# SudeepDasari/visual_foresight

Hardware: AMD Instinct MI355X
Metric: predicted frames/sec (whole node), 200-sample x 13-step x 64x64 CEM (higher is better)
Workload: dtype f32

## Files before the change

visual_foresight_amd/csrc/vf_conv_mfma.h:

```cpp
#pragma once
#include <hip/hip_runtime.h>
#include <type_traits>

#ifdef VF_HOST_SELFTEST
#define VF_GLOBAL __device__
#define VF_LAUNCH_BOUNDS(...)
#else
#define VF_GLOBAL __global__
#define VF_LAUNCH_BOUNDS(...) __launch_bounds__(__VA_ARGS__)
#endif

namespace vf {

constexpr int kPollSleep = 16;

#ifdef VF_TILE_STATS
__device__ unsigned long long g_tile_clk[32][8];
#define VF_TS_NOW() (threadIdx.x == 0 ? wall_clock64() : 0ull)
#define VF_TS_ADD(KEY_, SLOT_, DT_) do { if (threadIdx.x == 0) atomicAdd(&g_tile_clk[KEY_][SLOT_], (unsigned long long)(DT_)); } while (0)
#else
#define VF_TS_NOW() 0ull
#define VF_TS_ADD(KEY_, SLOT_, DT_) do { } while (0)
#endif

// ... 822 lines not shown
}

template <class PT>
__device__ __forceinline__ void conv_pair_epilogue(const PT &p, f32x16 (&acc)[1][2], const int bx, float *smem) {
    typedef const __attribute__((address_space(4))) ConvParams QT;
    const unsigned long long qa = reinterpret_cast<unsigned long long>(p.fuse_next);
    const unsigned qlo = __builtin_amdgcn_readfirstlane((unsigned)qa);
    const unsigned qhi = __builtin_amdgcn_readfirstlane((unsigned)(qa >> 32));
    QT &q = *(QT *)(((unsigned long long)qhi << 32) | qlo);
    const int tid = threadIdx.x, lane = tid & 63, wave = tid >> 6;
    const int n = lane & 31, kh = lane >> 5;
    constexpr int KCP = 36;
    const int bimg0 = bx * p.NI;
    float *T = smem;

    const int Ntot = q.ncg * 32;
    const float *wl = q.Wp + ((long long)kh * Ntot + n) * 4;
    const long long wstep = (long long)2 * Ntot * 4;
    f32x4 wb[2][4][2];
#pragma unroll
    for (int c = 0; c < 2; ++c)
#pragma unroll
        for (int k8 = 0; k8 < 4; ++k8)
#pragma unroll
            for (int g = 0; g < 2; ++g)
                wb[c][k8][g] = *reinterpret_cast<const f32x4 *>(wl + (long long)(c * 4 + k8) * wstep + g * 128);

    __syncthreads();
#pragma unroll
    for (int g = 0; g < 2; ++g) {
        const float bias = p.bias[g * 32 + n];
#pragma unroll
        for (int r = 0; r < 16; ++r) {
            const int row = wave * 32 + (r & 3) + 8 * (r >> 2) + 4 * kh;
            T[(g * 128 + row) * KCP + n] = fmaxf(acc[0][g][r] + bias, 0.f);
        }
    }
    __syncthreads();

    f32x16 acc2[2];
#pragma unroll
    for (int g = 0; g < 2; ++g)
#pragma unroll
        for (int r = 0; r < 16; ++r) acc2[g][r] = 0.f;
    const f32x4 *T4 = reinterpret_cast<const f32x4 *>(T);
    const int arow = wave * 32 + n;
#pragma unroll
    for (int c = 0; c < 2; ++c)
#pragma unroll
        for (int k8 = 0; k8 < 4; ++k8) {
            const f32x4 a = T4[((c * 128 + arow) * KCP + k8 * 8 + kh * 4) >> 2];
#pragma unroll
            for (int j = 0; j < 4; ++j)
#pragma unroll
                for (int g = 0; g < 2; ++g)
                    acc2[g] = __builtin_amdgcn_mfma_f32_32x32x2f32(a[j], wb[c][k8][g][j], acc2[g], 0, 0, 0);
        }

    const int px_per_img = q.TH * q.TW;
    const long long out_elems = (long long)q.Hout * q.Wout * q.Cout;
    const TileDiv div_rpi(q.RPI), div_tw(q.TW);
#pragma unroll
    for (int g = 0; g < 2; ++g) {
        const int ch = g * 32 + n;
        const float bias = q.bias[g * 32 + n];
#pragma unroll
        for (int r = 0; r < 16; ++r) {
            const int row = wave * 32 + (r & 3) + 8 * (r >> 2) + 4 * kh;
            const int img = div_rpi.div(row), rem = row - img * q.RPI;
            const int y = div_tw.div(rem), x = rem - y * q.TW;
            const int b = bimg0 + img;
            if (!(img < q.NI && rem < px_per_img && b < q.B && y < q.Hout && x < q.Wout && ch < q.Cout)) continue;
            float v = acc2[g][r] + bias;
            if (q.sbias) v += q.sbias[(long long)b * q.sbias_ld + ch];
            v = fmaxf(v, 0.f);
            (q.out + (long long)b * out_elems)[(unsigned)((y * q.Wout + x) * q.Cout + ch)] = v;
        }
    }
}

template <int ND, bool FIRST, int K, class PT>
__device__ __forceinline__ void convt_fused_epilogue(const PT &p, f32x16 (&acc)[1][4], int bx, long long *red, float *smem);

template <int G, int EPI, int MREP, class PT, int RB = 4>
__device__ __forceinline__ void conv_tile(const PT &p, const int bx_, const int by_, const int bz_,
                                          float *smem) {
    const int bx = __builtin_amdgcn_readfirstlane(bx_), by = __builtin_amdgcn_readfirstlane(by_),
              bz = __builtin_amdgcn_readfirstlane(bz_);
    constexpr bool SPLIT = RB == 1 || RB == 2;
    [[maybe_unused]] constexpr bool kInLaunch = !std::is_same<PT, ConvParams>::value;
    constexpr bool GSPLIT = RB <= 0;
    static_assert(RB == 4 || (G == 4 && EPI == EPI_LSTM && ((SPLIT && MREP == 1) || RB == 0 || (RB == -2 && MREP == 1))),
                  "the row-split and gate-split tiles are conv-LSTM tiles");
    constexpr int MR = RB == 0 ? 4 * MREP : (RB < 0 ? -RB : MREP);
    constexpr int WROWS = MR * 32;
    constexpr int GA = GSPLIT ? 1 : (SPLIT ? RB : G);
    constexpr bool kBRing = SPLIT && RB == 1;
    constexpr bool kBLds = (EPI == EPI_LSTM) && MREP == 1 && !kBRing && !GSPLIT;
    const int tid = threadIdx.x, lane = tid & 63, wave = tid >> 6;
    const int n = lane & 31, kh = lane >> 5;
    const int wrow0 = GSPLIT ? 0 : (SPLIT ? (wave % RB) * 32 : wave * WROWS);
    const int gbase = GSPLIT ? wave : (SPLIT ? (wave / RB) * GA : 0);
    const int KC = p.KC, KCpad = KC + 4, K8 = KC >> 3;
    const int LH = (p.TH - 1) * p.stride + p.KH, LW = (p.TW - 1) * p.stride + p.KW;
    const int tile_px = LH * LW;
    const int tile_floats = p.NI * tile_px * KCpad;
    float *lnTab = smem + tile_floats;
    long long *red = reinterpret_cast<long long *>(lnTab + 4 * p.NI);
    const int cg = by;
    const int tiles_per_img = p.tilesY * p.tilesX;

    int bimg0, ty0, tx0, tile_id;
    if (p.NI == 1) {
        bimg0 = bx / tiles_per_img;
        tile_id = bx % tiles_per_img;
        ty0 = (tile_id / p.tilesX) * p.TH;
        tx0 = (tile_id % p.tilesX) * p.TW;
    } else {
        bimg0 = bx * p.NI;
        tile_id = 0; ty0 = 0; tx0 = 0;
    }

    [[maybe_unused]] const unsigned long long ts0 = VF_TS_NOW();
    [[maybe_unused]] unsigned long long ts1 = 0, ts_stage = 0;
    [[maybe_unused]] int ts_key = (((p.seg[0].C + (p.nseg > 1 ? p.seg[1].C : 0)) >> 5) & 7) + (p.Hout >= 32 ? 0 : 8);
    if constexpr (EPI == EPI_RAW_STATS) ts_key = 16;
    else if constexpr (EPI == EPI_BIAS_RELU) ts_key = p.KH == 1 ? 17 : (p.seg[0].C == 32 ? 18 : 19);
    else if constexpr (EPI == EPI_CONVT_RELU) ts_key = p.nseg == 1 ? 20 : 21;
    else if constexpr (EPI == EPI_PARTIAL) ts_key = 22;
    else if constexpr (is_top_fused(EPI)) ts_key = 23;
    else if constexpr (EPI == EPI_CONVT_RAW_STATS) ts_key = 24;
    const bool late = p.late_cnt != nullptr;
    ln_table(p, bimg0, lnTab, 0, late ? 1 : 2);
    [[maybe_unused]] const bool yielding = kInLaunch && EPI == EPI_LSTM && (GSPLIT || (SPLIT && RB == 1)) && late &&
                                           p.cu_state != nullptr && p.yield_budget > 0;
    [[maybe_unused]] int ybudget = p.yield_budget;
    [[maybe_unused]] const int *yword = yielding ? cu_partner_word(p) : nullptr;

    const int px_per_img = p.TH * p.TW;
    int abase[MR];
    {
        const TileDiv div_rpi(p.RPI), div_tw(p.TW);
#pragma unroll
        for (int m = 0; m < MR; ++m) {
            const int row = wrow0 + m * 32 + n;
            const int img = div_rpi.div(row), rem = row - img * p.RPI;
            const bool ok = img < p.NI && rem < px_per_img;
            const int y = div_tw.div(rem), x = rem - y * p.TW;
            abase[m] = (ok ? (img * tile_px + y * p.stride * LW + x * p.stride) * KCpad : 0) + kh * 4;
        }
    }

    f32x16 acc[MR][GA];
#pragma unroll
    for (int m = 0; m < MR; ++m)
#pragma unroll
        for (int g = 0; g < GA; ++g)
#pragma unroll
            for (int r = 0; r < 16; ++r) acc[m][g][r] = 0.f;

    const int ntaps = p.KH * p.KW;
    const int Ntot = p.ncg * G * 32;
    const int total_chunks = p.seg[0].nchunk + (p.nseg > 1 ? p.seg[1].nchunk : 0);
    const int ch_begin = bz * p.chunks_per_split;
    const int ch_end = min(ch_begin + p.chunks_per_split, total_chunks);
    const float *wlane = p.Wp + ((long long)kh * Ntot + (cg * G) * 32 + n) * 4;
    const long long wstep = (long long)2 * Ntot * 4;

    const int q4 = KC >> 2;
    const int q4_log2 = 31 - __builtin_clz((unsigned)q4);
    const unsigned magic_px = 0xFFFFFFFFu / (unsigned)tile_px + 1u, magic_lw = 0xFFFFFFFFu / (unsigned)LW + 1u;
    const int items = p.NI * tile_px * q4;

    constexpr bool kGbTab = EPI == EPI_LSTM;
    const int gbC = kGbTab ? ((p.seg[0].C + (p.nseg > 1 ? p.seg[1].C : 0) + 3) & ~3) : 0;
    float *gbTab = lnTab + 4 * p.NI + 16;
    if constexpr (kGbTab) {
        for (int i = tid; i < gbC; i += kConvThreads) {
            const int sgi = i < p.seg[0].C ? 0 : 1;
            const int cc = sgi ? i - p.seg[0].C : i;
            float g = 1.f, b = 0.f;
            if (sgi < p.nseg && cc < p.seg[sgi].C && p.seg[sgi].ln_part) {
                const int m = cc % p.seg[sgi].gamma_mod;
                g = p.seg[sgi].gamma[m]; b = p.seg[sgi].beta[m];
            }
            gbTab[i] = g; gbTab[gbC + i] = b;
        }
    }
    f32x4 *bsm = reinterpret_cast<f32x4 *>(gbTab + 2 * gbC);
    const float *wgate = p.Wp + ((long long)kh * Ntot + (cg * G + (wave & (G - 1))) * 32 + n) * 4;
    const int gt0 = ch_begin * ntaps, gtN = ch_end * ntaps;
    f32x4 breg[4];
#define VF_LOADB(GT_)                                                                           \
    _Pragma("unroll") for (int q = 0; q < 4; ++q)                                               \
        if (q < K8) breg[q] = *reinterpret_cast<const f32x4 *>(wgate + ((long long)(GT_) * K8 + q) * wstep);
#define VF_WRITEB(BUF_)                                                                         \
    _Pragma("unroll") for (int q = 0; q < 4; ++q)                                               \
        if (q < K8) bsm[(((BUF_) * K8 + q) * 4 + wave) * 64 + lane] = breg[q];
    if constexpr (kBLds) {
        if (gt0 < gtN) { VF_LOADB(gt0) }
    }
    [[maybe_unused]] f32x4 gsA[GSPLIT ? 4 : 1], gsB[GSPLIT ? 4 : 1];
    [[maybe_unused]] int gs_par = 0;
    [[maybe_unused]] const unsigned gs_loff = (unsigned)(((kh * Ntot + (cg * G + wave) * 32 + n) * 4) * 4);
    [[maybe_unused]] const unsigned gs_wstep_b = (unsigned)wstep * 4u;
    [[maybe_unused]] const __amdgpu_buffer_rsrc_t gs_rsrc =
        __builtin_amdgcn_make_buffer_rsrc(const_cast<float *>(p.Wp), 0, 0x7FFFFFFF, 0x00020000);
    if constexpr (GSPLIT) {
        if (gt0 < gtN) {
#pragma unroll
            for (int q = 0; q < 4; ++q)
                gsA[q] = __builtin_bit_cast(f32x4, __builtin_amdgcn_raw_buffer_load_b128(
                    gs_rsrc, gs_loff, (unsigned)(gt0 * 4 + q) * gs_wstep_b, 0));
        }
    }
    constexpr int kRing = 5;
    [[maybe_unused]] f32x4 bring[kBRing ? kRing : 1][kBRing ? 4 : 1][GA];
    [[maybe_unused]] const float *wring = p.Wp + ((long long)kh * Ntot + (cg * G + gbase) * 32 + n) * 4;
#define VF_LOADRING(SLOT_, GT_)                                                                 \
    _Pragma("unroll") for (int q_ = 0; q_ < 4; ++q_)                                            \
        _Pragma("unroll") for (int g_ = 0; g_ < GA; ++g_)                                       \
            bring[SLOT_][q_][g_] = *reinterpret_cast<const f32x4 *>(                            \
                wring + ((long long)(GT_) * 4 + q_) * wstep + g_ * 128);
    if constexpr (kBRing) {
#pragma unroll
        for (int d = 0; d < kRing; ++d)
            if (gt0 + d < gtN) { VF_LOADRING(d, gt0 + d) }
    }

    constexpr bool kGRing = EPI != EPI_LSTM;
    constexpr bool kConvT = (EPI == EPI_CONVT_RELU || EPI == EPI_CONVT_RAW_STATS || is_top_fused(EPI));
    [[maybe_unused]] f32x4 gring[kGRing ? (G == 1 ? 5 : 4) : 1][G];
    [[maybe_unused]] const int nit_g = ntaps * K8;
    [[maybe_unused]] const int ring_d = (nit_g & 3) == 0 ? 4 : ((G == 1 && nit_g % 5 == 0) ? 5 : 0);
#define VF_TAPLIVE(TAP_) (kConvT ? ((((TAP_) >= p.KW) ? 15 : 3) & ((((TAP_) % p.KW) != 0) ? 15 : 5)) : 15)
    [[maybe_unused]] const unsigned gr_loff = (unsigned)(((kh * Ntot + (cg * G) * 32 + n) * 4) * 4);
    [[maybe_unused]] const unsigned gr_wstep_b = (unsigned)wstep * 4u;
    [[maybe_unused]] const __amdgpu_buffer_rsrc_t gr_rsrc =
        __builtin_amdgcn_make_buffer_rsrc(const_cast<float *>(p.Wp), 0, 0x7FFFFFFF, 0x00020000);
#define VF_GLOAD(SLOT_, CI_, IT_)                                                               \
    {                                                                                           \
        const unsigned so_ = (unsigned)((CI_) * nit_g + (IT_)) * gr_wstep_b;                    \
        _Pragma("unroll") for (int g_ = 0; g_ < G; ++g_)                                        \
            gring[SLOT_][g_] = __builtin_bit_cast(f32x4, __builtin_amdgcn_raw_buffer_load_b128( \
                gr_rsrc, gr_loff, so_ + 512u * g_, 0));                                          \
    }
    if constexpr (kGRing) {
        if (ch_begin < ch_end) {
            if (ring_d == 4) {
#pragma unroll
                for (int d = 0; d < 4; ++d) VF_GLOAD(d, ch_begin, d)
            } else if (G == 1 && ring_d == 5) {
#pragma unroll
                for (int d = 0; d < 5; ++d) VF_GLOAD(d, ch_begin, d)
            } else if (G == 2) {
#pragma unroll
                for (int d = 0; d < 2; ++d) VF_GLOAD(d, ch_begin, d)
            }
        }
    }

    if constexpr (EPI == EPI_LSTM) __builtin_amdgcn_s_setprio(0);
    constexpr int kStageU = 4;
    for (int ci = ch_begin; ci < ch_end; ++ci) {
        const int s = (ci < p.seg[0].nchunk) ? 0 : 1;
        const auto &sg = p.seg[s];
        const int c0 = (s == 0 ? ci : ci - p.seg[0].nchunk) * KC;
        const bool vec_ok = (sg.C & 3) == 0;

        if (late && ci == p.seg[0].nchunk) {
            const int b1 = p.NI == 1 ? bimg0 + 1 : min(bimg0 + p.NI, p.B);
            if constexpr (kInLaunch) VF_TRACE_EVT(TR_LATE);
            if (!late_wait(p, bimg0, b1, reinterpret_cast<int *>(red))) return;
            if constexpr (kInLaunch) VF_TRACE_EVT(TR_LATE_END);
            ln_table(p, bimg0, lnTab, 1, 2);
        }
        __syncthreads();
        if constexpr (kInLaunch) VF_TRACE_EVT(TR_STAGE);
        [[maybe_unused]] const unsigned long long ts_s0 = VF_TS_NOW();
        constexpr bool kHoistLn = EPI != EPI_LSTM || MREP > 1;
        const int q = tid & (q4 - 1);
        const int c = c0 + 4 * q;
        const int nvalid = min(4, sg.C - c);
        const bool lean = vec_ok && sg.C % KC == 0;
        [[maybe_unused]] float gam[4] = {1.f, 1.f, 1.f, 1.f}, bet[4] = {0.f, 0.f, 0.f, 0.f};
        if constexpr (kHoistLn) {
            if (sg.ln_part && c < sg.C && !(kGbTab && lean)) {
#pragma unroll
                for (int j = 0; j < 4; ++j) {
                    const int cc = (c + j) % sg.gamma_mod;
                    gam[j] = sg.gamma[cc]; bet[j] = sg.beta[cc];
                }
            }
        }
        bool staged = false;
        {
            if (lean) {
                staged = true;
                auto stage_fast = [&](auto ni1c) {
                    constexpr bool NI1 = decltype(ni1c)::value;
                    const int pl = tid >> q4_log2, ppp = kConvThreads >> q4_log2;
                    const bool has_ln = sg.ln_part != nullptr;
                    f32x4 gq = {1.f, 1.f, 1.f, 1.f}, bq = {0.f, 0.f, 0.f, 0.f};
                    if (has_ln) {
                        if constexpr (kGbTab) {
                            const int gi = (s == 0 ? 0 : p.seg[0].C) + c;
                            gq = *reinterpret_cast<const f32x4 *>(gbTab + gi);
                            bq = *reinterpret_cast<const f32x4 *>(gbTab + gbC + gi);
                        } else {
                            gq = f32x4{gam[0], gam[1], gam[2], gam[3]};
                            bq = f32x4{bet[0], bet[1], bet[2], bet[3]};
                        }
                    }
                    const int y0 = ty0 * p.stride - p.pad, x0 = tx0 * p.stride - p.pad;
                    const int npix = p.NI * tile_px;
                    const unsigned Cs = (unsigned)sg.C;
                    float mean1 = 0.f, rstd1 = 1.f;
                    if (NI1 && has_ln) { mean1 = lnTab[2 * s * p.NI]; rstd1 = lnTab[2 * s * p.NI + 1]; }
// ... 28 lines not shown
                        if constexpr (kInLaunch) { if (pix0 == pl) VF_TRACE_EVT(TR_ST_LOADED); }
#pragma unroll
                        for (int u = 0; u < kStageU; ++u) {
                            const int pix = pix0 + u * ppp;
                            if (pix >= npix) break;
                            if (oks[u]) {
                                if (has_ln) {
                                    float mean = mean1, rstd = rstd1;
                                    if constexpr (!NI1) {
                                        mean = lnTab[2 * (s * p.NI + imgs[u])];
                                        rstd = lnTab[2 * (s * p.NI + imgs[u]) + 1];
                                    }
#pragma unroll
                                    for (int j = 0; j < 4; ++j) v[u][j] = fmaf((v[u][j] - mean) * rstd, gq[j], bq[j]);
                                }
                                if (sg.relu) {
#pragma unroll
                                    for (int j = 0; j < 4; ++j) v[u][j] = fmaxf(v[u][j], 0.f);
                                }
                            }
                            *reinterpret_cast<f32x4 *>(dst + pix * KCpad) = v[u];
                        }
                    }
                };
                if (p.NI == 1) stage_fast(std::true_type{}); else stage_fast(std::false_type{});
            }
        }
        for (int it0 = tid; !staged && it0 < items; it0 += kConvThreads * kStageU) {
            f32x4 v[kStageU];
            int pixs[kStageU], imgs[kStageU];
            bool oks[kStageU];
#pragma unroll
            for (int u = 0; u < kStageU; ++u) {
                const int it = it0 + u * kConvThreads;
                const int pix = it >> q4_log2;
                const int img = tile_px == 1 ? pix : (int)__umulhi((unsigned)pix, magic_px), r = pix - img * tile_px;
                const int ly = LW == 1 ? r : (int)__umulhi((unsigned)r, magic_lw), lx = r - ly * LW;
                const int iy = ty0 * p.stride - p.pad + ly, ix = tx0 * p.stride - p.pad + lx;
                const int b = bimg0 + img;
                pixs[u] = pix; imgs[u] = img;
                oks[u] = it < items && b < p.B && iy >= 0 && iy < p.Hin && ix >= 0 && ix < p.Win && c < sg.C;
                v[u] = f32x4{0.f, 0.f, 0.f, 0.f};
                if (oks[u]) {
                    const float *src = sg.ptr + (long long)b * sg.bstride +
                                       ((long long)iy * p.Win + ix) * sg.C + c;
                    if (vec_ok) {
                        v[u] = *reinterpret_cast<const f32x4 *>(src);
                    } else {
#pragma unroll
                        for (int j = 0; j < 4; ++j) v[u][j] = (j < nvalid) ? src[j] : 0.f;
                    }
                }
            }
#pragma unroll
            for (int u = 0; u < kStageU; ++u) {
                if (it0 + u * kConvThreads >= items) break;
                if (oks[u]) {
                    if (sg.ln_part) {
                        const float mean = lnTab[2 * (s * p.NI + imgs[u])];
                        const float rstd = lnTab[2 * (s * p.NI + imgs[u]) + 1];
#pragma unroll
                        for (int j = 0; j < 4; ++j) {
                            if constexpr (kHoistLn) {
                                v[u][j] = fmaf((v[u][j] - mean) * rstd, gam[j], bet[j]);
                            } else {
                                const int cc = (c + j) % sg.gamma_mod;
                                v[u][j] = fmaf((v[u][j] - mean) * rstd, sg.gamma[cc], sg.beta[cc]);
                            }
                        }
                    }
                    if (sg.relu) {
#pragma unroll
                        for (int j = 0; j < 4; ++j) v[u][j] = fmaxf(v[u][j], 0.f);
                    }
#pragma unroll
                    for (int j = 0; j < 4; ++j) v[u][j] = (j < nvalid) ? v[u][j] : 0.f;
                }
                *reinterpret_cast<f32x4 *>(&smem[pixs[u] * KCpad + 4 * q]) = v[u];
            }
        }
        if constexpr (kBLds) {
            if (ci == ch_begin) { VF_WRITEB(0) }
        }
        if constexpr (kInLaunch) VF_TRACE_EVT(TR_ST_WRITTEN);
        __syncthreads();
#ifdef VF_TILE_STATS
        if (ci == ch_begin) ts1 = VF_TS_NOW(); else ts_stage += VF_TS_NOW() - ts_s0;
#endif
        if constexpr (kInLaunch) {
            if (ci == ch_begin) VF_TRACE_EVT(TR_MFMAS, (unsigned long long)(ntaps * K8 * 4 * GA * MR));
            VF_TRACE_EVT(TR_KLOOP);
        }

        const f32x4 *smem4 = reinterpret_cast<const f32x4 *>(smem);
        int ab4[MR];
#pragma unroll
        for (int m = 0; m < MR; ++m) ab4[m] = abase[m] >> 2;
        const int kcp4 = KCpad >> 2;
        [[maybe_unused]] f32x4 aP[GSPLIT ? 1 : MR], aQ[GSPLIT ? 1 : MR];
        [[maybe_unused]] f32x4 bP[GA], bQ[GA];
#define VF_MFMA(A_, B_)                                                                         \
        _Pragma("unroll") for (int j = 0; j < 4; ++j) {                                         \
            _Pragma("unroll") for (int g = 0; g < GA; ++g) {                                    \
                _Pragma("unroll") for (int m = 0; m < (GSPLIT ? 1 : MR); ++m)                   \
                    acc[m][g] = __builtin_amdgcn_mfma_f32_32x32x2f32(A_[m][j], B_[g][j], acc[m][g], 0, 0, 0); \
            }                                                                                   \
        }

        if constexpr (GSPLIT) {
            constexpr int GSZ = MR < 4 ? MR : 4;
            constexpr int NG = MR / GSZ, NS = 4 * NG;
            const f32x4 *ar[MR];
            f32x4 aP4[GSZ], aQ4[GSZ];
            auto gs_fetch = [&](f32x4 (&A_)[GSZ], const int kx, const int sub) {
#pragma unroll
                for (int m_ = 0; m_ < GSZ; ++m_) A_[m_] = ar[(sub % NG) * GSZ + m_][kx * 9 + (sub / NG) * 2];
            };
            auto gs_loadb = [&](f32x4 (&D_)[4], const int gt) {
                const unsigned so_ = (unsigned)(min(gt, gtN - 1) * 4) * gs_wstep_b;
#pragma unroll
                for (int q_ = 0; q_ < 4; ++q_)
                    D_[q_] = __builtin_bit_cast(f32x4, __builtin_amdgcn_raw_buffer_load_b128(
                        gs_rsrc, gs_loff, so_ + (unsigned)q_ * gs_wstep_b, 0));
            };
            auto gs_tap = [&](auto kxc, f32x4 (&cur)[4], f32x4 (&nxt)[4], const int gt_next) {
                constexpr int KX = decltype(kxc)::value;
                static_for<NS>([&](auto sc) {
                    constexpr int S = decltype(sc)::value;
                    f32x4 (&a_cur)[GSZ] = (S & 1) ? aQ4 : aP4;
                    f32x4 (&a_nxt)[GSZ] = (S & 1) ? aP4 : aQ4;
                    if constexpr (S + 1 < NS) gs_fetch(a_nxt, KX, S + 1);
                    else if constexpr (KX < 4) gs_fetch(a_nxt, KX + 1, 0);
                    __builtin_amdgcn_sched_barrier(0);
                    if constexpr (S == 0) {
                        gs_loadb(nxt, gt_next);
                        __builtin_amdgcn_sched_barrier(0);
                    }
                    const f32x4 bq = cur[S / NG];
#pragma unroll
                    for (int j_ = 0; j_ < 4; ++j_) {
#pragma unroll
                        for (int m_ = 0; m_ < GSZ; ++m_)
                            acc[(S % NG) * GSZ + m_][0] = __builtin_amdgcn_mfma_f32_32x32x2f32(
                                a_cur[m_][j_], bq[j_], acc[(S % NG) * GSZ + m_][0], 0, 0, 0);
                    }
                    __builtin_amdgcn_sched_barrier(0);
                });
            };
            const bool ychunk = yielding && ci < p.seg[0].nchunk;
            unsigned yseen = 0;
            auto gs_row = [&](f32x4 (&X_)[4], f32x4 (&Y_)[4], const int gt_row) {
                gs_fetch(aP4, 0, 0);
                gs_tap(std::integral_constant<int, 0>{}, X_, Y_, gt_row + 1);
                gs_tap(std::integral_constant<int, 1>{}, Y_, X_, gt_row + 2);
                gs_tap(std::integral_constant<int, 2>{}, X_, Y_, gt_row + 3);
                gs_tap(std::integral_constant<int, 3>{}, Y_, X_, gt_row + 4);
                gs_tap(std::integral_constant<int, 4>{}, X_, Y_, gt_row + 5);
            };
            for (int ky = 0; ky < 5; ++ky) {
                const int gt_row = ci * 25 + ky * 5;
                if (ychunk) yseen = yield_peek_issue(yword);
#pragma unroll
                for (int m = 0; m < MR; ++m) ar[m] = smem4 + ab4[m] + ky * LW * 9;
                if (gs_par == 0) gs_row(gsA, gsB, gt_row); else gs_row(gsB, gsA, gt_row);
                gs_par ^= 1;
                if (ychunk) yield_to_partner(yword, yseen, ybudget);
// ... 28 lines not shown
                        breg[q] = __builtin_bit_cast(f32x4, __builtin_amdgcn_raw_buffer_load_b128(
                            wrsrc, wl_off, (unsigned)((gt + 1) * 4 + q) * wstep_b, 0));
                }
                __builtin_amdgcn_sched_barrier(0);
                VF_MFMA(aP, bP)
                __builtin_amdgcn_sched_barrier(0);
                VF_FETCH_4(aP, bP, 2)
                __builtin_amdgcn_sched_barrier(0);
                VF_MFMA(aQ, bQ)
                __builtin_amdgcn_sched_barrier(0);
                VF_FETCH_4(aQ, bQ, 3)
                __builtin_amdgcn_sched_barrier(0);
                VF_MFMA(aP, bP)
                VF_MFMA(aQ, bQ)
                __builtin_amdgcn_sched_barrier(0);
#undef VF_FETCH_4
                if (more) {
                    f32x4 *bw = b_wr0 + (buf ^ 1) * (4 * 4 * 64);
#pragma unroll
                    for (int q = 0; q < 4; ++q) bw[q * 4 * 64] = breg[q];
                }
                __syncthreads();
                if (++kx == p.KW) { kx = 0; ++ky; }
            }
          } else {
#define VF_FETCH_L(A_, B_, Q_)                                                                  \
            {                                                                                   \
                _Pragma("unroll") for (int m = 0; m < MREP; ++m)                                \
                    A_[m] = smem4[ab4[m] + ao + (Q_) * 2];                            \
                _Pragma("unroll") for (int g = 0; g < GA; ++g)                                  \
                    B_[g] = bsm[((buf * K8 + (Q_)) * 4 + gbase + g) * 64 + lane];               \
            }
            for (int ky = 0; ky < p.KH; ++ky) {
                for (int kx = 0; kx < p.KW; ++kx) {
                    const int gt = ci * ntaps + ky * p.KW + kx;
                    const int buf = (gt - gt0) & 1;
                    const int ao = (ky * LW + kx) * kcp4;
                    const bool more = gt + 1 < gtN;
                    if (more) { VF_LOADB(gt + 1) }
                    VF_FETCH_L(aP, bP, 0)
                    int q = 0;
                    for (; q + 2 <= K8; q += 2) {
                        VF_FETCH_L(aQ, bQ, q + 1)
                        VF_MFMA(aP, bP)
                        if (q + 2 < K8) VF_FETCH_L(aP, bP, q + 2)
                        VF_MFMA(aQ, bQ)
                    }
                    if (q < K8) VF_MFMA(aP, bP)
                    if (more) { VF_WRITEB(buf ^ 1) }
                    __syncthreads();
                }
            }
#undef VF_FETCH_L
          }
        } else if constexpr (kBRing) {
            f32x4 aC[4], aN[4];
            const int a0 = ab4[0];
#pragma unroll
            for (int q = 0; q < 4; ++q) aC[q] = smem4[a0 + q * 2];
            const bool ychunk = yielding && ci < p.seg[0].nchunk;
            for (int ky = 0; ky < 5; ++ky) {
                unsigned yseen = 0;
                if (ychunk) yseen = yield_peek_issue(yword);
#pragma unroll
                for (int kx = 0; kx < kRing; ++kx) {
                    const int gt = ci * ntaps + ky * 5 + kx;
                    const int kyn = kx == 4 ? min(ky + 1, 4) : ky, kxn = kx == 4 ? (ky == 4 ? 4 : 0) : kx + 1;
                    const int aon = (kyn * LW + kxn) * kcp4;
#pragma unroll
                    for (int q = 0; q < 4; ++q) aN[q] = smem4[a0 + aon + q * 2];
#pragma unroll
                    for (int q = 0; q < 4; ++q)
#pragma unroll
                        for (int j = 0; j < 4; ++j)
#pragma unroll
                            for (int g = 0; g < GA; ++g)
                                acc[0][g] = __builtin_amdgcn_mfma_f32_32x32x2f32(aC[q][j], bring[kx][q][g][j], acc[0][g], 0, 0, 0);
                    if (gt + kRing < gtN) { VF_LOADRING(kx, gt + kRing) }
#pragma unroll
                    for (int q = 0; q < 4; ++q) aC[q] = aN[q];
                }
                if (ychunk) yield_to_partner(yword, yseen, ybudget);
            }
        } else if (kGRing && (G > 1 || ring_d != 0)) {
            auto kloop = [&](auto dc) {
                constexpr int D = decltype(dc)::value;
                f32x4 aC[MREP], aN[MREP];
                int ky = 0, kx = 0, k8 = 0;
                auto fetch_a = [&](f32x4 (&A_)[MREP]) {
                    const int ao_ = (ky * LW + kx) * kcp4 + k8 * 2;
#pragma unroll
                    for (int m = 0; m < MREP; ++m) A_[m] = smem4[ab4[m] + ao_];
                    if (++k8 == K8) { k8 = 0; if (++kx == p.KW) { kx = 0; ++ky; } }
                };
                fetch_a(aC);
                for (int it0 = 0; it0 < nit_g; it0 += D) {
#pragma unroll
                    for (int j = 0; j < D; ++j) {
                        const int it = it0 + j;
                        if (it + 1 < nit_g) fetch_a(aN);
                        const int live = VF_TAPLIVE(it / K8);
#pragma unroll
                        for (int g = 0; g < G; ++g) {
                            if (g == 0 || (live >> g) & 1) {
#pragma unroll
                                for (int jj = 0; jj < 4; ++jj)
#pragma unroll
                                    for (int m = 0; m < MREP; ++m)
                                        acc[m][g] = __builtin_amdgcn_mfma_f32_32x32x2f32(aC[m][jj], gring[j][g][jj], acc[m][g], 0, 0, 0);
                            }
                        }
                        const int nx = it + D;
                        if (nx < nit_g) { VF_GLOAD(j, ci, nx) }
                        else if (ci + 1 < ch_end) { VF_GLOAD(j, ci + 1, nx - nit_g) }
#pragma unroll
                        for (int m = 0; m < MREP; ++m) aC[m] = aN[m];
                    }
                }
            };
            if constexpr (G == 1) {
                if (ring_d == 4) kloop(std::integral_constant<int, 4>{});
                else kloop(std::integral_constant<int, 5>{});
            } else if constexpr (G == 2) {
                if (ring_d == 4) kloop(std::integral_constant<int, 4>{});
                else kloop(std::integral_constant<int, 2>{});
            } else {
                kloop(std::integral_constant<int, 4>{});
            }
        } else if constexpr (!(kGRing && G > 1)) {
            const float *wchunk = wlane + (long long)ci * ntaps * K8 * wstep;
            const int nit = ntaps * K8;
            int ky = 0, kx = 0, k8 = 0;
            [[maybe_unused]] int liveP = 15, liveQ = 15;
#define VF_FETCH(A_, B_, LIVE_, IT_)                                                            \
            {                                                                                   \
                const int ao_ = (ky * LW + kx) * kcp4 + k8 * 2;                                 \
                _Pragma("unroll") for (int m = 0; m < MREP; ++m) A_[m] = smem4[ab4[m] + ao_]; \
                const float *wp_ = wchunk + (long long)(IT_) * wstep;                             \
                if constexpr (kConvT) {                                                         \
                    LIVE_ = (ky ? 15 : 3) & (kx ? 15 : 5);                                      \
                    B_[0] = *reinterpret_cast<const f32x4 *>(wp_);                              \
                    if (LIVE_ & 2) B_[1 % G] = *reinterpret_cast<const f32x4 *>(wp_ + 128);     \
                    if (LIVE_ & 4) B_[2 % G] = *reinterpret_cast<const f32x4 *>(wp_ + 256);     \
                    if (LIVE_ & 8) B_[3 % G] = *reinterpret_cast<const f32x4 *>(wp_ + 384);     \
                } else {                                                                        \
                    _Pragma("unroll") for (int g = 0; g < G; ++g)                               \
                        B_[g] = *reinterpret_cast<const f32x4 *>(wp_ + g * 128);                \
                }                                                                               \
                if (++k8 == K8) { k8 = 0; if (++kx == p.KW) { kx = 0; ++ky; } }                 \
            }
#define VF_MFMA_G(A_, B_, G_)                                                                   \
            _Pragma("unroll") for (int j = 0; j < 4; ++j) {                                     \
                _Pragma("unroll") for (int m = 0; m < MREP; ++m)                                \
                    acc[m][(G_) % G] = __builtin_amdgcn_mfma_f32_32x32x2f32(A_[m][j], B_[(G_) % G][j], acc[m][(G_) % G], 0, 0, 0); \
            }
#define VF_MFMA_L(A_, B_, LIVE_)                                                                \
            if constexpr (kConvT) {                                                             \
                VF_MFMA_G(A_, B_, 0)                                                            \
                if (LIVE_ & 2) { VF_MFMA_G(A_, B_, 1) }                                         \
                if (LIVE_ & 4) { VF_MFMA_G(A_, B_, 2) }                                         \
                if (LIVE_ & 8) { VF_MFMA_G(A_, B_, 3) }                                         \
            } else {                                                                            \
                VF_MFMA(A_, B_)                                                                 \
            }
            VF_FETCH(aP, bP, liveP, 0)
            int it = 0;
            for (; it + 2 <= nit; it += 2) {
                VF_FETCH(aQ, bQ, liveQ, it + 1)
                VF_MFMA_L(aP, bP, liveP)
                if (it + 2 < nit) VF_FETCH(aP, bP, liveP, it + 2)
                VF_MFMA_L(aQ, bQ, liveQ)
            }
            if (it < nit) { VF_MFMA_L(aP, bP, liveP) }
#undef VF_FETCH
#undef VF_MFMA_G
#undef VF_MFMA_L
        }
#undef VF_MFMA
    }
#undef VF_LOADB
#undef VF_WRITEB
#undef VF_LOADRING
#undef VF_GLOAD
#undef VF_TAPLIVE

    if constexpr (EPI == EPI_LSTM) __builtin_amdgcn_s_setprio(2);
    if constexpr (kInLaunch) VF_TRACE_EVT(TR_EPI);
    [[maybe_unused]] const unsigned long long ts2 = VF_TS_NOW();
    if constexpr (GSPLIT) lstm_gsplit_epilogue<MR>(p, acc, bx, by, smem);
    else if constexpr (SPLIT && RB == 1) lstm_gsplit_epilogue<1>(p, acc, bx, by, smem);
    else if constexpr (SPLIT) lstm_split_epilogue<RB>(p, acc, bx, by, red, reinterpret_cast<float *>(bsm));
    else if constexpr (is_top_fused(EPI))
        convt_fused_epilogue<((EPI - EPI_CONVT_FUSED) & 7) / 2 + 1, ((EPI - EPI_CONVT_FUSED) & 1) != 0,
                             (EPI - EPI_CONVT_FUSED) >= 8 ? 6 : 10>(p, acc, bx, red, smem);
    else if constexpr (EPI == EPI_CONV_PAIR) conv_pair_epilogue(p, acc, bx, smem);
    else conv_epilogue<G, EPI, MREP>(p, acc, bx, by, bz, red, smem);
#ifdef VF_TILE_STATS
    {
        asm volatile("s_waitcnt vmcnt(0)" ::: "memory");
        const unsigned long long ts3 = VF_TS_NOW();
        VF_TS_ADD(ts_key, 0, ts1 - ts0); VF_TS_ADD(ts_key, 1, ts2 - ts1); VF_TS_ADD(ts_key, 2, ts3 - ts2);
        VF_TS_ADD(ts_key, 3, 1); VF_TS_ADD(ts_key, 4, ts_stage);
    }
#endif
}

template <int G, int EPI, int MREP>
VF_GLOBAL VF_LAUNCH_BOUNDS(kConvThreads, 2) void conv_mfma_kernel(const ConvParams p) {
    extern __shared__ __attribute__((aligned(16))) float smem[];
    conv_tile<G, EPI, MREP>(p, blockIdx.x, blockIdx.y, blockIdx.z, smem);
}

template <int RB>
VF_GLOBAL VF_LAUNCH_BOUNDS(kConvThreads, 2) void conv_lstm_split_kernel(const ConvParams p) {
    extern __shared__ __attribute__((aligned(16))) float smem[];
    conv_tile<4, EPI_LSTM, 1, ConvParams, RB>(p, blockIdx.x, blockIdx.y, 0, smem);
}

VF_GLOBAL VF_LAUNCH_BOUNDS(kConvThreads, 2) void conv_lstm_gsplit64_kernel(const ConvParams p) {
    extern __shared__ __attribute__((aligned(16))) float smem[];
    conv_tile<4, EPI_LSTM, 1, ConvParams, -2>(p, blockIdx.x, blockIdx.y, 0, smem);
}

template <int MREP>
VF_GLOBAL VF_LAUNCH_BOUNDS(kConvThreads, 2) void conv_lstm_gsplit_kernel(const ConvParams p) {
    extern __shared__ __attribute__((aligned(16))) float smem[];
    conv_tile<4, EPI_LSTM, MREP, ConvParams, 0>(p, blockIdx.x, blockIdx.y, 0, smem);
}

}
```

visual_foresight_amd/csrc/vf_engine.hip:

```cpp
#include <hip/hip_runtime.h>

#include <algorithm>
#include <cmath>
#include <cstdio>
#include <cstring>
#include <cstdlib>
#include <string>
#include <vector>

#include <dlfcn.h>
#ifdef VF_HOST_SELFTEST
#include <sys/mman.h>
#endif

#include "../../include/vf_hip.h"
#include "vf_conv_mfma.h"
#include "vf_small_kernels.h"
#include "vf_conv_bf16x6.h"
#include "vf_persistent.h"

#ifndef VF_WT_DEFAULT
#define VF_WT_DEFAULT 3
#endif

namespace vf {

static thread_local std::string g_last_error;

static int fail(int code, const std::string &msg) {
    g_last_error = msg;
    return code;
}

template <class R> static R api_error(int code);
template <> int api_error<int>(int code) { return code; }
template <> size_t api_error<size_t>(int) { return 0; }
template <> double api_error<double>(int) { return 0.0; }
#define VF_API_TRY try {
#define VF_API_CATCH_CLEANUP(RET_, CLEANUP_)                                                               \
    } catch (const std::bad_alloc &) {                                                                     \
        CLEANUP_                                                                                           \
        g_last_error.assign("out of memory");                                                              \
        return api_error<RET_>(VF_ERR_NOMEM);                                                              \
    } catch (const std::exception &e_) {                                                                   \
        CLEANUP_                                                                                           \
        try { g_last_error = std::string("exception: ") + e_.what(); } catch (...) { g_last_error.assign("exception"); } \
        return api_error<RET_>(VF_ERR_INVALID);                                                            \
    } catch (...) {                                                                                        \
        CLEANUP_                                                                                           \
        g_last_error.assign("unknown exception");                                                          \
        return api_error<RET_>(VF_ERR_INVALID);                                                            \
    }
#define VF_API_CATCH(RET_) VF_API_CATCH_CLEANUP(RET_, {})

#ifdef VF_HOST_SELFTEST
#include <stdexcept>
static int g_inject_where = 0, g_inject_kind = 0;
static void inject_point(int where) {
    if (g_inject_where != where) return;
    g_inject_where = 0;
    if (g_inject_kind == 0) throw std::bad_alloc();
    if (g_inject_kind == 1) throw std::runtime_error("injected failure");
    throw 42;
}
#define VF_INJECT(W_) inject_point(W_)
#else
#define VF_INJECT(W_) do { } while (0)
#endif

#define VF_HIP_CHECK(expr)                                                                  \
    do {                                                                                    \
        hipError_t err_ = (expr);                                                           \
        if (err_ != hipSuccess)                                                             \
            return fail(VF_ERR_HIP, std::string(#expr) + ": " + hipGetErrorString(err_));   \
    } while (0)

static const int kLstmSizes[7] = {32, 32, 64, 64, 128, 64, 32};
static const int kEnc00Ch = 16;
static const int kNumLn = 11;
static const int kSchedRing = 4;
static const int kTicketInts = kQueues * kTicketStride;
static const int kSyncHead = kTicketInts + kCuKeys * kCuWords;

struct TensorDesc {
    std::string name;
    int shape[4];
    int rank;
    size_t offset;
    size_t size() const {
// ... 37 lines not shown
    const int cc = c.arch == 2 ? a_of(c) : 0;
    const int Hc = savp ? c.height / 2 : c.height, Wc = savp ? c.width / 2 : c.width;
    const int fc_in = (Hc / 8) * (Wc / 8) * L[4];
    const bool pub = c.arch == 0 && c.layer_spec == 1;
    const int c_t2 = pub ? L[5] + L[1] : L[5], c_top = pub ? L[6] + 32 : 32;
    if (savp) { conv("enc00", 5, 5, 3, kEnc00Ch); ln("lna", kEnc00Ch); }
    conv("enc0", 5, 5, savp ? kEnc00Ch : 3, 32); ln("ln1", 32);
    conv("lstm1", 5, 5, 32 + cc + L[0], 4 * L[0]);  ln("ln2", L[0]);
    conv("lstm2", 5, 5, L[0] + cc + L[1], 4 * L[1]); ln("ln3", L[1]);
    conv("enc1", 3, 3, L[1], L[1]);
    conv("lstm3", 5, 5, L[1] + cc + L[2], 4 * L[2]); ln("ln4", L[2]);
    conv("lstm4", 5, 5, L[2] + cc + L[3], 4 * L[3]); ln("ln5", L[3]);
    conv("enc2", 3, 3, L[3], L[3]);
    conv("enc3", 1, 1, L[3] + a, L[3]);
    conv("lstm5", 5, 5, L[3] + cc + L[4], 4 * L[4]); ln("ln6", L[4]);
    conv("convt1", 3, 3, L[4], L[4]);
    conv("lstm6", 5, 5, L[4] + cc + L[5], 4 * L[5]); ln("ln7", L[5]);
    conv("convt2", 3, 3, L[5] + L[1], c_t2);
    conv("lstm7", 5, 5, c_t2 + cc + L[6], 4 * L[6]); ln("ln8", L[6]);
    conv("convt3", 3, 3, L[6] + 32, c_top);     ln("ln9", c_top);
    if (savp) { conv("convt4", 3, 3, 32 + kEnc00Ch, 32); ln("lnb", 32); }
    conv("rgb", 1, 1, c_top, 3);
    conv("masks", 1, 1, c_top, K + 1);
    const int KF = c.arch == 2 ? K - 2 : K;
    add("cdna/w", {fc_in, kTaps * KF});
    add("cdna/b", {kTaps * KF});
    add("state/w", {a, c.sdim});
    add("state/b", {c.sdim});
    return t;
}

static std::string ln_name(int i) { return i < 9 ? "ln" + std::to_string(i + 1) : (i == 9 ? "lna" : "lnb"); }

static const TensorDesc *find_tensor(const std::vector<TensorDesc> &t, const std::string &name) {
    for (const auto &d : t)
        if (d.name == name) return &d;
    return nullptr;
}

enum PackMode { PACK_PLAIN, PACK_LSTM, PACK_CONVT };
static const int kNumConvLayers = 24;

struct ConvLayer {
    std::string name;
    int id = -1;
    PackMode mode;
    int G;
    int Hin, Win, Hout, Wout;
    int KH, KW, stride, pad;
    int segC[2], nseg;
    int seg_off[2];
    int KC, nchunk[2];
    int mrep;
    int prec = 0;
    bool first_valu = false;
    bool gs_v2 = false;
    bool gsplit = false;
    int NI, TH, TW, RPI, tilesY, tilesX;
    int ni_cap = 0;
    int kc_cap = 0;
    int ncg, Cout;
    int nsplit, chunks_per_split, n_valid;
    int stats_nparts;
    size_t lds_bytes;
    size_t packed_w() const {
        if (first_valu) return (size_t)KH * KW * segC[0] * Cout;
        return (size_t)(nchunk[0] + nchunk[1]) * KH * KW * (KC / 8) * 2 * ((size_t)ncg * G * 32) * 4;
    }
    size_t packed_w16() const {
        return prec == 1 ? (size_t)(nchunk[0] + nchunk[1]) * KH * KW * ncg * 4 * 3 * 64 * 8 : 0;
    }
    size_t packed_b() const { return (size_t)ncg * G * 32; }
};

static bool top_fusable(const ConvLayer &l, int ND) {
    return l.NI == 1 && l.ncg == 1 && l.Cout == 32 && l.nsplit == 1 && l.TH * l.TW <= 128 &&
           (2 * l.TH) % kSumBlockH == 0 && (2 * l.TW) % kSumBlockW == 0 &&
           (2 * l.Hout) % kSumBlockH == 0 && (2 * l.Wout) % kSumBlockW == 0 &&
           fused_top_lds_floats(l.TH, l.TW, ND) * 4 <= 78 * 1024;
}

static int round_up(int x, int m) { return (x + m - 1) / m * m; }

static size_t conv_lds_bytes(const ConvLayer &l, int KC) {
    const int LH = (l.TH - 1) * l.stride + l.KH, LW = (l.TW - 1) * l.stride + l.KW;
    const size_t b_lds = (l.mode == PACK_LSTM && l.mrep <= 1) ? (size_t)2 * (KC / 8) * 4 * 64 * 16 : 0;
    const size_t gb_lds = l.mode == PACK_LSTM ? (size_t)2 * round_up(l.segC[0] + (l.nseg > 1 ? l.segC[1] : 0), 4) * 4 : 0;
    const size_t need = ((size_t)l.NI * LH * LW * (KC + 4) + 4 * (size_t)l.NI) * 4 + 64 + gb_lds + b_lds;
    return std::max(need, (size_t)vf::kEpiVecFloats * 4 + 64);
}

static void plan_geometry(ConvLayer &l, bool needs_stats, bool one_pixel_images) {
    const int rows = l.mrep == 0 ? 64 : (l.mrep < 0 ? 32 : 128 * l.mrep), wrows = l.mrep <= 0 ? 32 : 32 * l.mrep;
    if (one_pixel_images) {
        l.TH = l.TW = 1; l.tilesY = l.tilesX = 1; l.RPI = 1; l.NI = rows;
    } else {
        l.TW = std::min(l.Wout, 32);
        if (l.mode == PACK_LSTM && l.prec == 0 && l.mrep == 1 && l.KH == 5 && l.KW == 5) l.TW = std::min(l.Wout, 16);
#ifdef VF_DEBUG_KNOBS
        if (const char *e = getenv("VF_TILE_W")) l.TW = std::min(l.Wout, std::max(8, atoi(e)));
#endif
        l.TH = std::min(l.Hout, rows / l.TW);
        l.tilesX = (l.Wout + l.TW - 1) / l.TW;
        l.tilesY = (l.Hout + l.TH - 1) / l.TH;
        const int px = l.TH * l.TW;
        if (l.tilesX * l.tilesY == 1 && px <= rows / 2) {
            l.RPI = needs_stats ? round_up(px, wrows) : px;
            l.NI = rows / l.RPI;
            if (l.ni_cap > 0) l.NI = std::min(l.NI, l.ni_cap);
        } else {
            l.RPI = rows; l.NI = 1;
        }
    }
    const int maxC = std::max(l.segC[0], l.nseg > 1 ? l.segC[1] : 0);
    int KC = 32;
    while (KC > 8 && (KC > round_up(maxC, 8) || conv_lds_bytes(l, KC) > 78 * 1024 || (l.kc_cap > 0 && KC > l.kc_cap) ||
                      l.segC[0] % KC || (l.nseg > 1 && l.segC[1] % KC)))
        KC >>= 1;
    if (l.prec == 1) KC = kBfKC;
    l.KC = KC;
    for (int s = 0; s < 2; ++s) l.nchunk[s] = s < l.nseg ? (l.segC[s] + KC - 1) / KC : 0;
    l.lds_bytes = conv_lds_bytes(l, KC);
    bool gs256 = false;
#ifdef VF_DEBUG_KNOBS
    if (const char *e = getenv("VF_GSPLIT256")) gs256 = atoi(e) != 0;
#endif
    bool gs64 = true;
#ifdef VF_DEBUG_KNOBS
    if (const char *e = getenv("VF_GSPLIT64")) gs64 = atoi(e) != 0;
#endif
    l.gsplit = l.mode == PACK_LSTM && (l.mrep == 1 || (gs64 && l.mrep == 0) || (gs256 && l.mrep == 2 && l.NI == 1)) &&
               l.prec == 0 && KC == 32 && l.KH == 5 && l.KW == 5;
    l.gs_v2 = false;
    if (l.gsplit) {
        const size_t b_lds = l.mrep <= 1 ? (size_t)2 * (KC / 8) * 4 * 64 * 16 : 0;
        const int LH = (l.TH - 1) * l.stride + l.KH, LW = (l.TW - 1) * l.stride + l.KW;
        l.gs_v2 = l.mrep == 1 && l.stride == 1 && (size_t)l.NI * LH * LW <= 320;
#ifdef VF_DEBUG_KNOBS
        if (const char *e = getenv("VF_GSPLIT_V2")) l.gs_v2 = l.gs_v2 && atoi(e) != 0;
#else
        if (l.mrep == 1 && !l.gs_v2) l.gsplit = false;
#endif
        if (l.gsplit) l.lds_bytes = std::max(l.lds_bytes - b_lds, (size_t)vf::kGsXchFloats * 4 + 64);
    }
    if (l.prec == 1) {
        const int LH = (l.TH - 1) * l.stride + l.KH, LW = (l.TW - 1) * l.stride + l.KW;
        l.lds_bytes = bf16x6_lds_bytes(l.NI, LH, LW);
    }
    l.stats_nparts = (l.NI == 1 ? l.tilesY * l.tilesX : 1) * l.ncg;
}

static std::vector<float> pack_weights(const ConvLayer &l, const float *w, int KHc, int KWc, int Cin, int Ctot) {
    const int G = l.G, KC = l.KC, K8 = KC / 8, ntaps = l.KH * l.KW;
    const int Ntot = l.ncg * G * 32;
    const int nchunks = l.nchunk[0] + l.nchunk[1];
    std::vector<float> out((size_t)nchunks * ntaps * K8 * 2 * Ntot * 4, 0.f);
    for (int ci = 0; ci < nchunks; ++ci) {
        const int s = ci < l.nchunk[0] ? 0 : 1;
        const int c0 = (s == 0 ? ci : ci - l.nchunk[0]) * KC;
        const int seg_off = l.seg_off[s];
        for (int ty = 0; ty < l.KH; ++ty)
            for (int tx = 0; tx < l.KW; ++tx)
                for (int k8 = 0; k8 < K8; ++k8)
                    for (int kh = 0; kh < 2; ++kh)
                        for (int col = 0; col < Ntot; ++col) {
                            const int cgi = col / (G * 32), g = (col / 32) % G, nn = col % 32;
                            const int co = cgi * 32 + nn;
                            if (co >= l.Cout) continue;
                            int ky = ty, kx = tx, ocol;
                            if (l.mode == PACK_LSTM) {
                                ocol = g * l.Cout + co;
                            } else if (l.mode == PACK_CONVT) {
                                ky = (g >> 1) + 2 * (1 - ty);
                                kx = (g & 1) + 2 * (1 - tx);
                                if (ky >= KHc || kx >= KWc) continue;
                                ocol = co;
                            } else {
                                ocol = co;
                            }
                            for (int j = 0; j < 4; ++j) {
                                const int c = c0 + k8 * 8 + kh * 4 + j;
                                if (c >= l.segC[s]) continue;
                                const int cin = seg_off + c;
                                const size_t dst = ((((((size_t)ci * ntaps + (ty * l.KW + tx)) * K8 + k8) * 2 + kh) * Ntot + col) * 4) + j;
                                out[dst] = w[(((size_t)ky * KWc + kx) * Cin + cin) * Ctot + ocol];
                            }
                        }
    }
    return out;
}

static unsigned short bf16_rne(float x) {
    unsigned u;
    memcpy(&u, &x, 4);
    if ((u & 0x7f800000u) == 0x7f800000u) return (unsigned short)(u >> 16);
    u += 0x7fffu + ((u >> 16) & 1u);
    return (unsigned short)(u >> 16);
}
static float bf16_to_f32(unsigned short h) {
    unsigned u = (unsigned)h << 16;
    float x;
    memcpy(&x, &u, 4);
    return x;
// ... 2375 lines not shown
```

Baseline: 41730.

## Stage transposed-conv weights in LDS and specialize the parity-sparse MFMA loop

```diff
diff --git a/visual_foresight_amd/csrc/vf_conv_mfma.h b/visual_foresight_amd/csrc/vf_conv_mfma.h
--- a/visual_foresight_amd/csrc/vf_conv_mfma.h
+++ b/visual_foresight_amd/csrc/vf_conv_mfma.h
@@ -928,6 +928,9 @@
 template <int ND, bool FIRST, int K, class PT>
 __device__ __forceinline__ void convt_fused_epilogue(const PT &p, f32x16 (&acc)[1][4], int bx, long long *red, float *smem);
 
+__host__ __device__ constexpr int convt_live(const int tap) { return (tap >= 2 ? 15 : 3) & ((tap & 1) ? 15 : 5); }
+__host__ __device__ constexpr int convt_slot0(const int tap) { return tap == 0 ? 0 : 2 * tap - 1; }
+
 template <int G, int EPI, int MREP, class PT, int RB = 4>
 __device__ __forceinline__ void conv_tile(const PT &p, const int bx_, const int by_, const int bz_,
                                           float *smem) {
@@ -943,6 +946,8 @@
     constexpr int GA = GSPLIT ? 1 : (SPLIT ? RB : G);
     constexpr bool kBRing = SPLIT && RB == 1;
     constexpr bool kBLds = (EPI == EPI_LSTM) && MREP == 1 && !kBRing && !GSPLIT;
+    constexpr bool kConvT = (EPI == EPI_CONVT_RELU || EPI == EPI_CONVT_RAW_STATS || is_top_fused(EPI));
+    static_assert(!kConvT || (G == 4 && MREP == 1 && RB == 4), "transposed convs: 4 parities, 128-row tiles");
     const int tid = threadIdx.x, lane = tid & 63, wave = tid >> 6;
     const int n = lane & 31, kh = lane >> 5;
     const int wrow0 = GSPLIT ? 0 : (SPLIT ? (wave % RB) * 32 : wave * WROWS);
@@ -1074,12 +1079,44 @@
             if (gt0 + d < gtN) { VF_LOADRING(d, gt0 + d) }
     }
 
-    constexpr bool kGRing = EPI != EPI_LSTM;
-    constexpr bool kConvT = (EPI == EPI_CONVT_RELU || EPI == EPI_CONVT_RAW_STATS || is_top_fused(EPI));
+    constexpr bool kTLds = kConvT;
+    constexpr int kTSlots = 9, kTPerWave = (kTSlots * 4 + 3) / 4;
+    constexpr unsigned long long kTSlotTap = 0x333322110ull, kTSlotPar = 0x321020100ull;
+    [[maybe_unused]] f32x4 treg[kTLds ? kTPerWave : 1];
+    [[maybe_unused]] const int wave_s = __builtin_amdgcn_readfirstlane(wave);
+    [[maybe_unused]] const int k8_log2 = 31 - __builtin_clz((unsigned)K8);
+    [[maybe_unused]] const unsigned tl_loff = (unsigned)(((kh * Ntot + (cg * G) * 32 + n) * 4) * 4);
+    [[maybe_unused]] const unsigned tl_wstep_b = (unsigned)wstep * 4u;
+    [[maybe_unused]] const __amdgpu_buffer_rsrc_t tl_rsrc =
+        __builtin_amdgcn_make_buffer_rsrc(const_cast<float *>(p.Wp), 0, 0x7FFFFFFF, 0x00020000);
+    [[maybe_unused]] unsigned tl_voff[kTLds ? kTPerWave : 1];
+    if constexpr (kTLds) {
+#pragma unroll
+        for (int i = 0; i < kTPerWave; ++i) {
+            const int b = wave_s + 4 * i, sl = min(b >> k8_log2, kTSlots - 1);
+            const int tap = (int)((kTSlotTap >> (4 * sl)) & 15), g = (int)((kTSlotPar >> (4 * sl)) & 15);
+            tl_voff[i] = tl_loff + (unsigned)(tap * K8 + (b & (K8 - 1))) * tl_wstep_b + 512u * g;
+        }
+    }
+#define VF_TLOAD(CI_)                                                                           \
+    _Pragma("unroll") for (int i_ = 0; i_ < kTPerWave; ++i_) {                                  \
+        if (wave_s + 4 * i_ < kTSlots * K8)                                                     \
+            treg[i_] = __builtin_bit_cast(f32x4, __builtin_amdgcn_raw_buffer_load_b128(        \
+                tl_rsrc, tl_voff[i_], (unsigned)((CI_) * 4 * K8) * tl_wstep_b, 0));             \
+    }
+#define VF_TWRITE()                                                                             \
+    _Pragma("unroll") for (int i_ = 0; i_ < kTPerWave; ++i_) {                                  \
+        const int b_ = wave_s + 4 * i_;                                                         \
+        if (b_ < kTSlots * K8) bsm[(((b_ >> k8_log2) << 2) + (b_ & (K8 - 1))) * 64 + lane] = treg[i_]; \
+    }
+    if constexpr (kTLds) {
+        if (ch_begin < ch_end) { VF_TLOAD(ch_begin) }
+    }
+
+    constexpr bool kGRing = EPI != EPI_LSTM && !kConvT;
     [[maybe_unused]] f32x4 gring[kGRing ? (G == 1 ? 5 : 4) : 1][G];
     [[maybe_unused]] const int nit_g = ntaps * K8;
     [[maybe_unused]] const int ring_d = (nit_g & 3) == 0 ? 4 : ((G == 1 && nit_g % 5 == 0) ? 5 : 0);
-#define VF_TAPLIVE(TAP_) (kConvT ? ((((TAP_) >= p.KW) ? 15 : 3) & ((((TAP_) % p.KW) != 0) ? 15 : 5)) : 15)
     [[maybe_unused]] const unsigned gr_loff = (unsigned)(((kh * Ntot + (cg * G) * 32 + n) * 4) * 4);
     [[maybe_unused]] const unsigned gr_wstep_b = (unsigned)wstep * 4u;
     [[maybe_unused]] const __amdgpu_buffer_rsrc_t gr_rsrc =
@@ -1274,6 +1311,7 @@
         if constexpr (kBLds) {
             if (ci == ch_begin) { VF_WRITEB(0) }
         }
+        if constexpr (kTLds) { VF_TWRITE() }
         if constexpr (kInLaunch) VF_TRACE_EVT(TR_ST_WRITTEN);
         __syncthreads();
 #ifdef VF_TILE_STATS
@@ -1468,6 +1506,52 @@
                 }
                 if (ychunk) yield_to_partner(yword, yseen, ybudget);
             }
+        } else if constexpr (kTLds) {
+            if (ci + 1 < ch_end) { VF_TLOAD(ci + 1) }
+            const f32x4 *a0 = smem4 + ab4[0], *a1 = a0 + LW * kcp4;
+            const f32x4 *bt = bsm + lane;
+            f32x4 aP, aQ, bP[4], bQ[4];
+            auto fetch = [&](auto tc, auto qc, f32x4 &A_, f32x4 (&B_)[4], auto nbc) {
+                constexpr int T = decltype(tc)::value, Q = decltype(qc)::value, nl = __builtin_popcount(convt_live(T));
+                A_ = (T < 2 ? a0 : a1)[(T & 1) * kcp4 + Q * 2];
+#pragma unroll
+                for (int r = 0; r < decltype(nbc)::value; ++r) B_[r] = bt[((convt_slot0(T) + min(r, nl - 1)) * 4 + Q) * 64];
+            };
+            using I0 = std::integral_constant<int, 0>;
+            auto nb = [](auto tc) { return std::integral_constant<int, __builtin_popcount(convt_live(decltype(tc)::value))>{}; };
+            fetch(I0{}, I0{}, aP, bP, nb(I0{}));
+            static_for<16>([&](auto sc) {
+                constexpr int S = decltype(sc)::value, T = S / 4, Q = S % 4;
+                f32x4 &a_cur = (Q & 1) ? aQ : aP, &a_nxt = (Q & 1) ? aP : aQ;
+                f32x4 (&b_cur)[4] = (Q & 1) ? bQ : bP;
+                f32x4 (&b_nxt)[4] = (Q & 1) ? bP : bQ;
+                if (Q < K8) {
+                    using TN = std::integral_constant<int, T + 1>;
+                    using TC = std::integral_constant<int, T>;
+                    if constexpr (Q == 1 && T < 3) {
+                        using NB = std::integral_constant<int, std::max(decltype(nb(TC{}))::value, decltype(nb(TN{}))::value)>;
+                        if (K8 == 4) fetch(TC{}, std::integral_constant<int, 2>{}, a_nxt, b_nxt, NB{});
+                        else fetch(TN{}, I0{}, a_nxt, b_nxt, NB{});
+                    } else if constexpr (Q == 1) {
+                        if (K8 == 4) fetch(TC{}, std::integral_constant<int, 2>{}, a_nxt, b_nxt, nb(TC{}));
+                    } else if constexpr (Q < 3) {
+                        fetch(TC{}, std::integral_constant<int, Q + 1>{}, a_nxt, b_nxt, nb(TC{}));
+                    } else if constexpr (T < 3) {
+                        fetch(TN{}, I0{}, a_nxt, b_nxt, nb(TN{}));
+                    }
+                    __builtin_amdgcn_sched_barrier(0);
+                    static_for<4>([&](auto gc) {
+                        constexpr int g = decltype(gc)::value;
+                        if constexpr ((convt_live(T) >> g) & 1) {
+                            constexpr int r = __builtin_popcount(convt_live(T) & ((1 << g) - 1));
+#pragma unroll
+                            for (int j = 0; j < 4; ++j)
+                                acc[0][g] = __builtin_amdgcn_mfma_f32_32x32x2f32(a_cur[j], b_cur[r][j], acc[0][g], 0, 0, 0);
+                        }
+                    });
+                    __builtin_amdgcn_sched_barrier(0);
+                }
+            });
         } else if (kGRing && (G > 1 || ring_d != 0)) {
             auto kloop = [&](auto dc) {
                 constexpr int D = decltype(dc)::value;
@@ -1485,16 +1569,13 @@
                     for (int j = 0; j < D; ++j) {
                         const int it = it0 + j;
                         if (it + 1 < nit_g) fetch_a(aN);
-                        const int live = VF_TAPLIVE(it / K8);
 #pragma unroll
                         for (int g = 0; g < G; ++g) {
-                            if (g == 0 || (live >> g) & 1) {
-#pragma unroll
-                                for (int jj = 0; jj < 4; ++jj)
-#pragma unroll
-                                    for (int m = 0; m < MREP; ++m)
-                                        acc[m][g] = __builtin_amdgcn_mfma_f32_32x32x2f32(aC[m][jj], gring[j][g][jj], acc[m][g], 0, 0, 0);
-                            }
+#pragma unroll
+                            for (int jj = 0; jj < 4; ++jj)
+#pragma unroll
+                                for (int m = 0; m < MREP; ++m)
+                                    acc[m][g] = __builtin_amdgcn_mfma_f32_32x32x2f32(aC[m][jj], gring[j][g][jj], acc[m][g], 0, 0, 0);
                         }
                         const int nx = it + D;
                         if (nx < nit_g) { VF_GLOAD(j, ci, nx) }
@@ -1517,50 +1598,25 @@
             const float *wchunk = wlane + (long long)ci * ntaps * K8 * wstep;
             const int nit = ntaps * K8;
             int ky = 0, kx = 0, k8 = 0;
-            [[maybe_unused]] int liveP = 15, liveQ = 15;
-#define VF_FETCH(A_, B_, LIVE_, IT_)                                                            \
+#define VF_FETCH(A_, B_, IT_)                                                                   \
             {                                                                                   \
                 const int ao_ = (ky * LW + kx) * kcp4 + k8 * 2;                                 \
                 _Pragma("unroll") for (int m = 0; m < MREP; ++m) A_[m] = smem4[ab4[m] + ao_]; \
                 const float *wp_ = wchunk + (long long)(IT_) * wstep;                             \
-                if constexpr (kConvT) {                                                         \
-                    LIVE_ = (ky ? 15 : 3) & (kx ? 15 : 5);                                      \
-                    B_[0] = *reinterpret_cast<const f32x4 *>(wp_);                              \
-                    if (LIVE_ & 2) B_[1 % G] = *reinterpret_cast<const f32x4 *>(wp_ + 128);     \
-                    if (LIVE_ & 4) B_[2 % G] = *reinterpret_cast<const f32x4 *>(wp_ + 256);     \
-                    if (LIVE_ & 8) B_[3 % G] = *reinterpret_cast<const f32x4 *>(wp_ + 384);     \
-                } else {                                                                        \
-                    _Pragma("unroll") for (int g = 0; g < G; ++g)                               \
-                        B_[g] = *reinterpret_cast<const f32x4 *>(wp_ + g * 128);                \
-                }                                                                               \
+                _Pragma("unroll") for (int g = 0; g < G; ++g)                                   \
+                    B_[g] = *reinterpret_cast<const f32x4 *>(wp_ + g * 128);                    \
                 if (++k8 == K8) { k8 = 0; if (++kx == p.KW) { kx = 0; ++ky; } }                 \
             }
-#define VF_MFMA_G(A_, B_, G_)                                                                   \
-            _Pragma("unroll") for (int j = 0; j < 4; ++j) {                                     \
-                _Pragma("unroll") for (int m = 0; m < MREP; ++m)                                \
-                    acc[m][(G_) % G] = __builtin_amdgcn_mfma_f32_32x32x2f32(A_[m][j], B_[(G_) % G][j], acc[m][(G_) % G], 0, 0, 0); \
-            }
-#define VF_MFMA_L(A_, B_, LIVE_)                                                                \
-            if constexpr (kConvT) {                                                             \
-                VF_MFMA_G(A_, B_, 0)                                                            \
-                if (LIVE_ & 2) { VF_MFMA_G(A_, B_, 1) }                                         \
-                if (LIVE_ & 4) { VF_MFMA_G(A_, B_, 2) }                                         \
-                if (LIVE_ & 8) { VF_MFMA_G(A_, B_, 3) }                                         \
-            } else {                                                                            \
-                VF_MFMA(A_, B_)                                                                 \
-            }
-            VF_FETCH(aP, bP, liveP, 0)
+            VF_FETCH(aP, bP, 0)
             int it = 0;
             for (; it + 2 <= nit; it += 2) {
-                VF_FETCH(aQ, bQ, liveQ, it + 1)
-                VF_MFMA_L(aP, bP, liveP)
-                if (it + 2 < nit) VF_FETCH(aP, bP, liveP, it + 2)
-                VF_MFMA_L(aQ, bQ, liveQ)
-            }
-            if (it < nit) { VF_MFMA_L(aP, bP, liveP) }
+                VF_FETCH(aQ, bQ, it + 1)
+                VF_MFMA(aP, bP)
+                if (it + 2 < nit) VF_FETCH(aP, bP, it + 2)
+                VF_MFMA(aQ, bQ)
+            }
+            if (it < nit) { VF_MFMA(aP, bP) }
 #undef VF_FETCH
-#undef VF_MFMA_G
-#undef VF_MFMA_L
         }
 #undef VF_MFMA
     }
@@ -1568,7 +1624,8 @@
 #undef VF_WRITEB
 #undef VF_LOADRING
 #undef VF_GLOAD
-#undef VF_TAPLIVE
+#undef VF_TLOAD
+#undef VF_TWRITE
 
     if constexpr (EPI == EPI_LSTM) __builtin_amdgcn_s_setprio(2);
     if constexpr (kInLaunch) VF_TRACE_EVT(TR_EPI);
diff --git a/visual_foresight_amd/csrc/vf_engine.hip b/visual_foresight_amd/csrc/vf_engine.hip
--- a/visual_foresight_amd/csrc/vf_engine.hip
+++ b/visual_foresight_amd/csrc/vf_engine.hip
@@ -5,6 +5,7 @@
 #include <cstdio>
 #include <cstring>
 #include <cstdlib>
+#include <stdexcept>
 #include <string>
 #include <vector>
 
@@ -208,9 +209,12 @@
 
 static int round_up(int x, int m) { return (x + m - 1) / m * m; }
 
+static size_t convt_b_lds_bytes() { return (size_t)9 * 4 * 64 * 16; }
+
 static size_t conv_lds_bytes(const ConvLayer &l, int KC) {
     const int LH = (l.TH - 1) * l.stride + l.KH, LW = (l.TW - 1) * l.stride + l.KW;
-    const size_t b_lds = (l.mode == PACK_LSTM && l.mrep <= 1) ? (size_t)2 * (KC / 8) * 4 * 64 * 16 : 0;
+    const size_t b_lds = (l.mode == PACK_LSTM && l.mrep <= 1) ? (size_t)2 * (KC / 8) * 4 * 64 * 16
+                                                               : (l.mode == PACK_CONVT ? convt_b_lds_bytes() : 0);
     const size_t gb_lds = l.mode == PACK_LSTM ? (size_t)2 * round_up(l.segC[0] + (l.nseg > 1 ? l.segC[1] : 0), 4) * 4 : 0;
     const size_t need = ((size_t)l.NI * LH * LW * (KC + 4) + 4 * (size_t)l.NI) * 4 + 64 + gb_lds + b_lds;
     return std::max(need, (size_t)vf::kEpiVecFloats * 4 + 64);
@@ -240,11 +244,16 @@
     }
     const int maxC = std::max(l.segC[0], l.nseg > 1 ? l.segC[1] : 0);
     int KC = 32;
-    while (KC > 8 && (KC > round_up(maxC, 8) || conv_lds_bytes(l, KC) > 78 * 1024 || (l.kc_cap > 0 && KC > l.kc_cap) ||
+    auto operand_lds = [&](int kc) { return conv_lds_bytes(l, kc) - (l.mode == PACK_CONVT ? convt_b_lds_bytes() : 0); };
+    while (KC > 8 && (KC > round_up(maxC, 8) || operand_lds(KC) > 78 * 1024 || (l.kc_cap > 0 && KC > l.kc_cap) ||
                       l.segC[0] % KC || (l.nseg > 1 && l.segC[1] % KC)))
         KC >>= 1;
     if (l.prec == 1) KC = kBfKC;
     l.KC = KC;
+    if (l.mode == PACK_CONVT) {
+        if (KC < 16) throw std::invalid_argument("transposed conv " + l.name + ": channel counts must be multiples of 16");
+        while (l.NI > 1 && conv_lds_bytes(l, KC) > 78 * 1024) --l.NI;
+    }
     for (int s = 0; s < 2; ++s) l.nchunk[s] = s < l.nseg ? (l.segC[s] + KC - 1) / KC : 0;
     l.lds_bytes = conv_lds_bytes(l, KC);
     bool gs256 = false;
```

Measured after the change: 41750 (median of 5 runs). Within noise of the previous version (+0.0%).
